# RuyiLian/CheckerPose

Measured on AMD Instinct MI355X. Metric: crops/sec forward (256x256, npt=512), higher is better.
Workload: dtype bf16; 1 GPU; LMO 'ape' hr18GNN2_res6_gnn3Skip_mlpQuery npt=512, PoseNet_GNNskip forward, deterministic random-init weights; global_batch=256, parallelism=dp1 (no forward collective), launch=hipGraph replay of 104 kernel launches

## Files before the change

### __graft_entry__.py

```python
import os
import subprocess
import sys

ROOT = os.path.dirname(os.path.abspath(__file__))
if ROOT not in sys.path:
    sys.path.insert(0, ROOT)


def build():
    csrc = os.path.join(ROOT, "checkerpose_amd", "csrc")
    subprocess.check_call(["make", "-C", csrc, "-j4", "ARCH=gfx950"])
    import checkerpose_amd
    from checkerpose_amd import _abi
    lib = _abi.load()
    assert lib.cp_version() >= 233


def smoke():
    import torch
    from oracle import checkerpose_oracle as O
    from checkerpose_amd.synthetic import build_net, det_image
    oracle_kwargs = lambda: dict(backbone="hrnet_w18", res_log2=6, init_n_graph=2, n_graph=3, local_k=2, slope=0.01,
                                 graph_slope=0.2, init_graph_slope=0.2)
    assert torch.cuda.is_available(), "smoke() needs an MI355X"
    torch.set_grad_enabled(False)
    net = build_net(seed=1)
    img = det_image(1, seed=0)
    ref, _ = O.posenet_forward(net.state_dict(), img, net.init_net.knn_idx, 512, **oracle_kwargs())
    net = net.cuda()
    out = net(img.cuda(), None)
    torch.cuda.synchronize()
    worst = 0.0
    for a, b in zip(out[:4], ref[:4]):
        worst = max(worst, float((a.cpu() - b).abs().max()))
    ids_ok = bool((out[4].cpu() == ref[4]).all() and (out[5].cpu() == ref[5]).all())
    print("smoke: max |logit - oracle| = %.3e, ids equal = %s" % (worst, ids_ok))
    assert worst <= 1e-4, worst
    assert ids_ok


if __name__ == "__main__":
    build()
    if len(sys.argv) > 1 and sys.argv[1] == "smoke":
        smoke()
```

### checkerpose_amd/_abi.py

```python
import ctypes as C
import os

_HERE = os.path.dirname(os.path.abspath(__file__))
LIB_PATH = os.environ.get("CHECKERPOSE_AMD_LIB") or os.path.join(_HERE, "libcheckerpose_hip.so")

CP_F32, CP_BF16, CP_F16 = 0, 1, 2
ACT_NONE, ACT_RELU, ACT_LEAKY = 0, 1, 2
LOSS_BCE, LOSS_L1 = 0, 1
POSE_ERR_ADD, POSE_ERR_ADI = 1, 2
BOP_ERR_MSSD, BOP_ERR_MSPD, BOP_ERR_PROJ, BOP_MAP_SMALL, BOP_MAP_LARGE = 1, 2, 4, 16, 32
BOP_MATCH_NO_LDS, BOP_MATCH_SCRATCH_MASK, BOP_SCORES_NO_LDS = 1, 2, 1


class CpConvDesc(C.Structure):
    _fields_ = [("dtype", C.c_int32), ("out_f32", C.c_int32), ("B", C.c_int32), ("H", C.c_int32), ("W", C.c_int32),
                ("Cin", C.c_int32), ("in_cstride", C.c_int32), ("in_coff", C.c_int32),
                ("R", C.c_int32), ("S", C.c_int32), ("stride", C.c_int32), ("pad", C.c_int32),
                ("Ho", C.c_int32), ("Wo", C.c_int32), ("Cout", C.c_int32), ("act", C.c_int32), ("slope", C.c_float), ("ksplit", C.c_int32),
                ("o_base", C.c_int64), ("o_sb", C.c_int64), ("o_sy", C.c_int64), ("o_sx", C.c_int64),
                ("o_sc", C.c_int64)]


_P, _I, _F, _L = C.c_void_p, C.c_int, C.c_float, C.c_longlong

# ... 30 lines not shown
                ("dw_sr", C.c_int64), ("dw_ss", C.c_int64)]


CP_BN_ITEM_STATS, CP_BN_ITEM_APPLY, CP_BN_ITEM_BWD_SUMS, CP_BN_ITEM_BWD_APPLY = 0, 1, 2, 3
BN_GROUP_MAX = 16


class CpBnItem(C.Structure):
    _fields_ = [("kind", C.c_int32), ("dtype", C.c_int32), ("blocks", C.c_uint32), ("lds_bytes", C.c_uint32),
                ("params", C.c_uint64 * 24)]


CP_WGRAD_ITEM_3X3, CP_WGRAD_ITEM_3X3_SMALL, CP_WGRAD_ITEM_GENERIC_BF16, CP_WGRAD_ITEM_GENERIC_F32 = 0, 1, 2, 3
CP_WGRAD_ITEM_3X3_S2_SMALL = 4


class CpWgradItem(C.Structure):
    _fields_ = [("kind", C.c_int32), ("blocks", C.c_uint32), ("gx", C.c_uint32), ("gy", C.c_uint32), ("params", C.c_uint64 * 20)]


class CpOptItem(C.Structure):
    _fields_ = [("p", C.c_void_p), ("g", C.c_void_p), ("m", C.c_void_p), ("v", C.c_void_p), ("n", C.c_uint64), ("step0", C.c_uint32),
                ("pad", C.c_uint32)]


class CpFuseBwdItem(C.Structure):
    _fields_ = [("dout", C.c_void_p), ("out", C.c_void_p), ("dsrc", C.c_void_p), ("Hs", C.c_int32), ("Ws", C.c_int32), ("CG", C.c_int32),
                ("shift", C.c_int32), ("relu", C.c_int32), ("accumulate", C.c_int32), ("total", C.c_uint64)]


class CpWgradDesc(C.Structure):
    _fields_ = [("dtype", C.c_int32), ("B", C.c_int32), ("H", C.c_int32), ("W", C.c_int32), ("Ho", C.c_int32),
                ("Wo", C.c_int32), ("Cout", C.c_int32), ("dy_cstride", C.c_int32), ("dy_coff", C.c_int32),
                ("Cin", C.c_int32), ("x_cstride", C.c_int32), ("x_coff", C.c_int32),
                ("R", C.c_int32), ("S", C.c_int32), ("stride", C.c_int32), ("pad", C.c_int32),
                ("dw_base", C.c_int64), ("dw_sco", C.c_int64), ("dw_sci", C.c_int64), ("dw_sr", C.c_int64),
                ("dw_ss", C.c_int64)]


SIGNATURES = {
    "cp_version": (_I, []),
    "cp_device_status": (_I, [_P, _I]),
    "cp_set_deterministic": (None, [_I]),
    "cp_get_deterministic": (_I, []),
    "cp_strerror": (C.c_char_p, [_I]),
    "cp_last_kernel": (C.c_char_p, []),
    "cp_kernel_log_begin": (None, []),
    "cp_kernel_log": (C.c_char_p, []),
    "cp_chan_align": (_I, [_I]),
    "cp_packed_weight_bytes": (C.c_size_t, [_I, _I, _I, _I, _I]),
    "cp_pack_conv_weight": (_I, [_P, _I, _P, _I, _I, _I, _I, _I, _I, _I, _P, _I, _P]),
    "cp_conv2d_igemm": (_I, [_P, C.POINTER(CpConvDesc), _P, _P, _P, _P, _P, _P]),
    "cp_conv2d_igemm_splitk": (_I, [_I, C.c_longlong, _I, _I]),
    "cp_packed_halo_weight_bytes": (C.c_size_t, [_I, _I, _I]),
    "cp_pack_conv3x3_halo_weight": (_I, [_P, _I, _P, _I, _I, _I, _P]),
    "cp_conv3x3_halo": (_I, [_P, C.POINTER(CpConvDesc), _P, _P, _P, _P, _P, _P]),
    "cp_conv2x2_halo_supported": (_I, [_I, _I, _I, _I]),
    "cp_packed_conv2x2_halo_weight_bytes": (C.c_size_t, [_I, _I, _I]),
    "cp_pack_conv2x2_halo_weight": (_I, [_P, _I, _P, _I, _I, _I, _P]),
    "cp_conv2x2_halo": (_I, [_P, C.POINTER(CpConvDesc), _P, _P, _P, _P, _P, _P]),
    "cp_conv3x3_s2_small_supported": (_I, [_I, _I, _I, _I]),
    "cp_conv3x3_s2_small_weight_bytes": (C.c_size_t, [_I, _I]),
    "cp_pack_conv3x3_s2_small_weight": (_I, [_P, _P, _I, _I, _I, _I, _P]),
    "cp_conv3x3_s2_small": (_I, [_P, C.POINTER(CpConvDesc), _P, _P, _P, _P, _P]),
    "cp_conv3x3_halo_up2x_supported": (_I, [_I, _I]),
    "cp_conv3x3_halo_up2x": (_I, [_P, C.POINTER(CpConvDesc), _P, _P, _P, _P, _P]),
    "cp_conv3x3_halo_seg_supported": (_I, [_I, _I, _I]),
    "cp_conv3x3_halo_seg": (_I, [_P, C.POINTER(CpConvDesc), _P, _P, _P, _P, _P, _P, _P, _I, _P]),
    "cp_pack_conv3x3_rows_weight": (_I, [_P, _I, _P, _I, _I, _I, _P]),
    "cp_basicblock_fused": (_I, [_P, C.POINTER(CpConvDesc), _P, _P, _P, _P, _P, _P, _P, _P]),
    "cp_bottleneck_fused": (_I, [_P, C.POINTER(CpConvDesc)] + [_P] * 14),
    "cp_packed_gemm_weight_bytes": (C.c_size_t, [_I, _I, _I]),
    "cp_pack_gemm_weight": (_I, [_P, _I, _P, _I, _I, _I, _P]),
    "cp_gemm_rows": (_I, [_P, C.POINTER(CpConvDesc), _P, _P, _P, _P, _P, _P]),
    "cp_mlp_query_fused_supported": (_I, [_I, _I, _I, _I]),
    "cp_mlp_query_fused": (_I, [_P, _P, _I, _I, _I, _I, _P, _P, _P, _F, _P, _P, _P, _F, _P, _P, _P, _L, _L, _L, _L]),
    "cp_mlp_query_fused_t": (_I, [_P, _I, _P, _I, _I, _I, _I, _P, _P, _P, _F, _P, _P, _P, _F, _P, _P, _P, _L, _L, _L, _L]),
    "cp_mlp_query_fused_n": (_I, [_P, _I, _P, _I, _I, _I, _I, _P, _P, _P, _F, _P, _P, _P, _F, _P, _P, _I, _P, _L, _L, _L, _L,
                                  _P, _P, _P, _P]),
    "cp_mlp_pair_fused_supported": (_I, [_I, _I, _I]),
    "cp_mlp_pair_fused": (_I, [_P, _P, _I, _I, _I, _I, _I, _P, _P, _F, _P, _P, _F, _P, _I, _I]),
    "cp_mlp_pair_fused_t": (_I, [_P, _I, _P, _I, _I, _I, _I, _I, _P, _P, _F, _P, _P, _F, _P, _I, _I]),
    "cp_mlp_pair_fused_gather_supported": (_I, [_I, _I, _I]),
    "cp_mlp_pair_fused_gather": (_I, [_P, C.POINTER(CpI2fGather), _P, _I, _I, _I, _I, _I, _P, _P, _F, _P, _P, _F, _P, _I, _I]),
    "cp_mlp_pair_fused_gather_t": (_I, [_P, _I, C.POINTER(CpI2fGather), _P, _I, _I, _I, _I, _I, _P, _P, _F, _P, _P, _F, _P, _I, _I]),
    "cp_hr_stem_weight_bytes": (C.c_size_t, [_I]),
    "cp_pack_hr_stem_weights": (_I, [_P, _P, _P, _P, _P]),
    "cp_hr_stem": (_I, [_P, _P, _I, _I, _I, _P, _P, _P, _P, _P, _P, _P]),
    "cp_hr_chain_supported": (_I, [_I, _I, _I]),
    "cp_hr_chain_weight_bytes": (C.c_size_t, [_I, _I, _I]),
    "cp_hr_chain_affine_floats": (_I, [_I, _I, _I]),
    "cp_pack_hr_chain_weight": (_I, [_P, _P, _P, _I, _I, _I, _I, _P]),
    "cp_hr_branch_chain": (_I, [_P, _I, _I, _I, _I, _I, C.POINTER(_P), C.POINTER(C.c_int32), _I, _P, _P, _P]),
    "cp_hr_chain_tail_supported": (_I, [_I, _I, _I]),
    "cp_hr_chain_tail_weight_bytes": (C.c_size_t, []),
    "cp_hr_chain_tail_channels": (_I, []),
    "cp_pack_hr_chain_tail_weight": (_I, [_P, _P, _P, _I, _I, _I, _P]),
    "cp_hr_branch_chain_tail": (_I, [_P, _I, _I, _I, _I, _I, C.POINTER(_P), C.POINTER(C.c_int32), _I, _P, _P, _P, C.POINTER(CpChainTail)]),
    "cp_hr_chain_tailconv_supported": (_I, [_I, _I, _I, _I, _I]),
    "cp_hr_chain_tailconv_weight_bytes": (C.c_size_t, [_I, _I, _I, _I, _I]),
    "cp_pack_hr_chain_tailconv_weight": (_I, [_P, _P, _P, _I, _I, _I, _I, _I, _P]),
    "cp_hr_branch_chain_tails": (_I, [_P, _I, _I, _I, _I, _I, C.POINTER(_P), C.POINTER(C.c_int32), _I, _P, _P, _P, _I, C.POINTER(CpChainTailConv)]),
    "cp_upsample2x_bilinear_ac": (_I, [_P, _I, _P, _P, _I, _I, _I, _I, _I, _I, _I, _I]),
    "cp_fuse_sum_act": (_I, [_P, _I, _I, C.POINTER(_P), C.POINTER(C.c_int32), _P, _I, _I, _I, _I, _I, _I, _I]),
    "cp_maxpool3x3s2": (_I, [_P, _I, _P, _P, _I, _I, _I, _I]),
    "cp_edgeconv_gather_max": (_I, [_P, _I, _P, _P, _P, _P, _I, _I, _I, _I, _I, _I, _I, _F]),
# ... 235 lines not shown
```

### checkerpose_amd/csrc/api.hip

```cpp
#include <stdarg.h>
#include <stdio.h>
#include <string.h>

#include "common.h"

extern "C" int cp_version(void) { return 233; }

std::atomic<int> g_cp_deterministic{0};
extern "C" void cp_set_deterministic(int on) { g_cp_deterministic.store(on ? 1 : 0, std::memory_order_relaxed); }
extern "C" int cp_get_deterministic(void) { return g_cp_deterministic.load(std::memory_order_relaxed); }

static std::atomic<uint32_t*> g_status_word[256];
uint32_t* cp_status_word(bool create) {
  const int dev = cp_current_device();
  if (dev < 0 || dev > 255) return nullptr;
  uint32_t* p = g_status_word[dev].load(std::memory_order_acquire);
  if (p || !create) return p;
  hipStreamCaptureStatus cs = hipStreamCaptureStatusNone;
  if (hipStreamIsCapturing(nullptr, &cs) == hipSuccess && cs != hipStreamCaptureStatusNone) return nullptr;
  uint32_t* q = nullptr;
  if (hipMalloc((void**)&q, 256) != hipSuccess) return nullptr;
  if (hipMemset(q, 0, 256) != hipSuccess) { (void)hipFree(q); return nullptr; }
  uint32_t* expect = nullptr;
  if (!g_status_word[dev].compare_exchange_strong(expect, q, std::memory_order_acq_rel)) { (void)hipFree(q); return expect; }
  return q;
}
extern "C" int cp_device_status(uint32_t* status_out, int clear) {
  if (!status_out) return CP_ERR_INVALID;
  uint32_t* p = cp_status_word(true);
  if (!p) return CP_ERR_HIP;
  if (hipMemcpy(status_out, p, sizeof(uint32_t), hipMemcpyDeviceToHost) != hipSuccess) return CP_ERR_HIP;
  if (clear && *status_out && hipMemset(p, 0, sizeof(uint32_t)) != hipSuccess) return CP_ERR_HIP;
  return CP_OK;
}

static thread_local char g_last_kernel[128] = "";
static thread_local char g_kernel_log[1024] = "";
void cp_mark_kernel(const char* fmt, ...) {
  char tmp[128];
  va_list ap;
  va_start(ap, fmt);
  vsnprintf(tmp, sizeof(tmp), fmt, ap);
  va_end(ap);
  const char* b = tmp;
  size_t n = strlen(tmp);
  if (n >= 2 && tmp[0] == '(' && tmp[n - 1] == ')') { b = tmp + 1; n -= 2; }
  memcpy(g_last_kernel, b, n);
  g_last_kernel[n] = 0;
  const size_t have = strlen(g_kernel_log);
  if (have + n + 4 < sizeof(g_kernel_log))
    snprintf(g_kernel_log + have, sizeof(g_kernel_log) - have, "%s%s", have ? " + " : "", g_last_kernel);
}
extern "C" const char* cp_last_kernel(void) { return g_last_kernel; }
extern "C" void cp_kernel_log_begin(void) { g_kernel_log[0] = 0; }
extern "C" const char* cp_kernel_log(void) { return g_kernel_log; }

extern "C" const char* cp_strerror(int code) {
  switch (code) {
    case CP_OK: return "ok";
// ... 34 lines not shown
```

### checkerpose_amd/csrc/conv_igemm.hip

```cpp
#include <stdlib.h>

#include "common.h"

struct ConvParams {
  const void* in; const void* w; const float* scale; const float* shift; const void* res; void* out;
  int M, H, W, HoWo, Wo;
  int Cin, in_cs, in_coff;
  int R, S, stride, pad;
  int KC, Cout, n_tiles, m_blocks, n_blocks, old_map;
  int act; float slope; int out_f32; int epi_lds;
  uint32_t in_bytes, w_bytes;
  long long o_base, o_sb, o_sy, o_sx, o_sc;
};

template <typename Tag> struct Mma;
template <> struct Mma<F32Tag> {
  static __device__ __forceinline__ void run(const u32x4& w, const u32x4& a, f32x4& acc) {
    acc = __builtin_amdgcn_mfma_f32_16x16x4f32(__uint_as_float(w.x), __uint_as_float(a.x), acc, 0, 0, 0);
    acc = __builtin_amdgcn_mfma_f32_16x16x4f32(__uint_as_float(w.y), __uint_as_float(a.y), acc, 0, 0, 0);
    acc = __builtin_amdgcn_mfma_f32_16x16x4f32(__uint_as_float(w.z), __uint_as_float(a.z), acc, 0, 0, 0);
    acc = __builtin_amdgcn_mfma_f32_16x16x4f32(__uint_as_float(w.w), __uint_as_float(a.w), acc, 0, 0, 0);
  }
};
template <> struct Mma<BF16Tag> {
  static __device__ __forceinline__ void run(const u32x4& w, const u32x4& a, f32x4& acc) {
    acc = __builtin_amdgcn_mfma_f32_16x16x32_bf16(__builtin_bit_cast(bf16x8, w), __builtin_bit_cast(bf16x8, a), acc, 0, 0, 0);
  }
};

template <> struct Mma<F16Tag> {
  static __device__ __forceinline__ void run(const u32x4& w, const u32x4& a, f32x4& acc) { acc = cp_mma16<true>(w, a, acc); }
};

template <typename Tag, int MT, int NT>
__global__ __launch_bounds__(256) void conv_igemm_kernel(const ConvParams p) {
  if (p.out_f32 == 2 || Tag::dtype == CP_F16) cp_f16_saturate_on();
  constexpr int E = Tag::E;
  constexpr int KCH = 4 * E;
  constexpr int ES = 16 / E;
  const int lane = threadIdx.x & 63;
  const int wave = __builtin_amdgcn_readfirstlane(threadIdx.x >> 6);
  const int x = lane & 15, q = lane >> 4;
  const int label = blockIdx.x & 7, slot = blockIdx.x >> 3;
  int nblk = slot % p.n_blocks;
  int mblk = (slot / p.n_blocks) * 8 + label;
  if (p.old_map) { const int m8 = (p.m_blocks + 7) / 8 * 8; mblk = blockIdx.x % m8; nblk = blockIdx.x / m8; }
  if (mblk >= p.m_blocks) return;
  const int m_wave = mblk * (4 * MT * 16) + wave * (MT * 16);
  const int nt0 = nblk * NT;

  int iy0[MT], ix0[MT], rowbase[MT];
#pragma unroll
  for (int mt = 0; mt < MT; ++mt) {
    const int m = m_wave + mt * 16 + x;
    const bool ok = m < p.M;
    const int mm = ok ? m : 0;
    const int b = mm / p.HoWo;
    const int rem = mm - b * p.HoWo;
    const int oy = rem / p.Wo;
    const int ox = rem - oy * p.Wo;
    iy0[mt] = ok ? oy * p.stride - p.pad : -(1 << 28);
    ix0[mt] = ox * p.stride - p.pad;
    rowbase[mt] = ((b * p.H + (ok ? iy0[mt] : 0)) * p.W + ix0[mt]) * p.in_cs + p.in_coff;
  }
  int kk = q * E;
  int tap = kk / p.Cin;
  int c = kk - tap * p.Cin;
  int r = tap / p.S;
  int s = tap - r * p.S;

  const __amdgpu_buffer_rsrc_t rsrc =
      __builtin_amdgcn_make_buffer_rsrc(const_cast<void*>(p.in), 0, p.in_bytes, 0x00020000);
  const __amdgpu_buffer_rsrc_t wrsrc =
      __builtin_amdgcn_make_buffer_rsrc(const_cast<void*>(p.w), 0, p.w_bytes, 0x00020000);
  uint32_t woff[NT];
#pragma unroll
  for (int nt = 0; nt < NT; ++nt) {
    int t = nt0 + nt;
    t = t < p.n_tiles ? t : p.n_tiles - 1;
    woff[nt] = ((uint32_t)t * p.KC * 64 + lane) * 16u;
  }

  constexpr bool EPI = (MT == 2 && (NT == 1 || NT == 2 || NT == 4));
  constexpr bool f32o = (E == 4);
  constexpr int CPL = f32o ? 4 : 8;
  constexpr int LPP = EPI ? NT * 16 / CPL : 1;
  constexpr int PPP = 64 / LPP;
  constexpr int NPASS = EPI ? MT * 16 / PPP : 1;
  const int pl0 = lane / LPP, cg = lane - pl0 * LPP;
  const int cch = nt0 * 16 + cg * CPL;
  u32x4 rres[NPASS];
  long long ofs[NPASS];
  bool okp[NPASS];
  if constexpr (EPI) if (p.epi_lds) {
    const bool cok = cch < p.Cout;
#pragma unroll
    for (int ps = 0; ps < NPASS; ++ps) {
      const int m = m_wave + ps * PPP + pl0;
      okp[ps] = (m < p.M) & cok;
      const int mm = m < p.M ? m : 0;
      const int b = mm / p.HoWo;
      const int rem = mm - b * p.HoWo;
      const int oy = rem / p.Wo;
      const int ox = rem - oy * p.Wo;
      ofs[ps] = p.o_base + (long long)b * p.o_sb + (long long)oy * p.o_sy + (long long)ox * p.o_sx + cch;
      rres[ps] = u32x4{0u, 0u, 0u, 0u};
      if (p.res && okp[ps])
        rres[ps] = f32o ? *(const u32x4*)((const float*)p.res + ofs[ps]) : *(const u32x4*)((const uint16_t*)p.res + ofs[ps]);
    }
  }

  f32x4 acc[MT][NT];
#pragma unroll
  for (int mt = 0; mt < MT; ++mt)
#pragma unroll
    for (int nt = 0; nt < NT; ++nt) acc[mt][nt] = f32x4{0.f, 0.f, 0.f, 0.f};

  const bool wide_c = p.Cin >= KCH;
  auto load_chunk = [&](u32x4* a, u32x4* w, int kc) {
    const int tapoff = (r * p.W + s) * p.in_cs + c;
    const bool tap_ok = r < p.R;
#pragma unroll
    for (int mt = 0; mt < MT; ++mt) {
      const bool ok = tap_ok & ((unsigned)(iy0[mt] + r) < (unsigned)p.H) & ((unsigned)(ix0[mt] + s) < (unsigned)p.W);
      const uint32_t off = ok ? (uint32_t)(rowbase[mt] + tapoff) * ES : 0x80000000u;
      a[mt] = __builtin_bit_cast(u32x4, __builtin_amdgcn_raw_buffer_load_b128(rsrc, off, 0, 0));
    }
#pragma unroll
    for (int nt = 0; nt < NT; ++nt)
      w[nt] = __builtin_bit_cast(u32x4, __builtin_amdgcn_raw_buffer_load_b128(wrsrc, woff[nt] + (uint32_t)kc * 1024u, 0, 0));
    c += KCH;
    if (wide_c) {
      const bool wrap = c >= p.Cin;
      c = wrap ? c - p.Cin : c;
      s += wrap ? 1 : 0;
      const bool swrap = s == p.S;
      s = swrap ? 0 : s;
      r += swrap ? 1 : 0;
    } else {
      while (c >= p.Cin) {
        c -= p.Cin;
        if (++s == p.S) { s = 0; ++r; }
      }
    }
  };
  auto compute = [&](const u32x4* a, const u32x4* w) {
#pragma unroll
    for (int mt = 0; mt < MT; ++mt)
#pragma unroll
      for (int nt = 0; nt < NT; ++nt) Mma<Tag>::run(w[nt], a[mt], acc[mt][nt]);
  };

  u32x4 a0[MT], w0[NT], a1[MT], w1[NT];
  load_chunk(a0, w0, 0);
  load_chunk(a1, w1, 1);
  for (int kc = 0; kc < p.KC; kc += 2) {
    compute(a0, w0);
    load_chunk(a0, w0, kc + 2);
    if (kc + 1 < p.KC) compute(a1, w1);
    load_chunk(a1, w1, kc + 3);
  }

  if constexpr (EPI) if (p.epi_lds) {
    extern __shared__ __attribute__((aligned(16))) float epi_smem[];
    constexpr int ROWF = NT * 16 + 4;
    float* my = epi_smem + wave * (MT * 16 * ROWF);
#pragma unroll
    for (int mt = 0; mt < MT; ++mt)
#pragma unroll
      for (int nt = 0; nt < NT; ++nt) {
        const int n = (nt0 + nt) * 16 + q * 4;
        f32x4 v = f32x4{0.f, 0.f, 0.f, 0.f};
        if (nt0 + nt < p.n_tiles && n < p.Cout) {
          const f32x4 sc = *(const f32x4*)(p.scale + n);
          const f32x4 sh = *(const f32x4*)(p.shift + n);
#pragma unroll
          for (int j = 0; j < 4; ++j) v[j] = acc[mt][nt][j] * sc[j] + sh[j];
        }
        *(f32x4*)(my + (mt * 16 + x) * ROWF + nt * 16 + q * 4) = v;
      }
    __builtin_amdgcn_s_waitcnt(0xc07f);
    __builtin_amdgcn_wave_barrier();
#pragma unroll
    for (int ps = 0; ps < NPASS; ++ps) {
      const float* src = my + (ps * PPP + pl0) * ROWF + cg * CPL;
      float v[8];
      const f32x4 v0 = *(const f32x4*)src;
      v[0] = v0[0]; v[1] = v0[1]; v[2] = v0[2]; v[3] = v0[3];
      if (!f32o) { const f32x4 v1 = *(const f32x4*)(src + 4); v[4] = v1[0]; v[5] = v1[1]; v[6] = v1[2]; v[7] = v1[3]; }
      if (!okp[ps]) continue;
      if (p.res) {
        if (f32o) {
          v[0] += __uint_as_float(rres[ps].x); v[1] += __uint_as_float(rres[ps].y);
          v[2] += __uint_as_float(rres[ps].z); v[3] += __uint_as_float(rres[ps].w);
        } else {
          float r8[8];
          Vec16<BF16Tag>::unpack(rres[ps], r8);
#pragma unroll
          for (int j = 0; j < 8; ++j) v[j] += r8[j];
        }
      }
#pragma unroll
      for (int j = 0; j < 8; ++j) {
        v[j] = cp_act_apply(v[j], cp_act_slope(p.act, p.slope));
      }
      if (f32o) *(f32x4*)((float*)p.out + ofs[ps]) = f32x4{v[0], v[1], v[2], v[3]};
      else *(u32x4*)((uint16_t*)p.out + ofs[ps]) = Vec16<BF16Tag>::pack(v);
    }
    return;
  }

  const bool vec = (p.o_sc == 1);
  const bool f32io = p.out_f32 == 1 || E == 4;
  const bool h16out = p.out_f32 == 2 || (Tag::dtype == CP_F16 && p.out_f32 == 0);
  long long pix[MT];
  bool pok[MT];
#pragma unroll
  for (int mt = 0; mt < MT; ++mt) {
    const int m = m_wave + mt * 16 + x;
// ... 22 lines not shown
                               __uint_as_float(r2.y << 16), __uint_as_float(r2.y & 0xffff0000u)};
          }
        }
      }
  }
#pragma unroll
  for (int mt = 0; mt < MT; ++mt) {
    if (!pok[mt]) continue;
#pragma unroll
    for (int nt = 0; nt < NT; ++nt) {
      const int n = (nt0 + nt) * 16 + q * 4;
      if (nt0 + nt >= p.n_tiles || n >= p.Cout) continue;
      const f32x4 sc = *(const f32x4*)(p.scale + n);
      const f32x4 sh = *(const f32x4*)(p.shift + n);
      float v[4];
#pragma unroll
      for (int j = 0; j < 4; ++j) v[j] = acc[mt][nt][j] * sc[j] + sh[j];
      if (vec) {
        const long long o = pix[mt] + n;
        if (p.res) {
#pragma unroll
          for (int j = 0; j < 4; ++j) v[j] += rv[mt][nt][j];
        }
#pragma unroll
        for (int j = 0; j < 4; ++j) {
          v[j] = cp_act_apply(v[j], cp_act_slope(p.act, p.slope));
        }
        if (f32io) {
          *(f32x4*)((float*)p.out + o) = f32x4{v[0], v[1], v[2], v[3]};
        } else if (h16out) {
          u32x2 pk; pk.x = cp_pack2<true>(v[0], v[1]); pk.y = cp_pack2<true>(v[2], v[3]);
          *(u32x2*)((uint16_t*)p.out + o) = pk;
        } else {
          u32x2 pk; pk.x = pack_bf16x2(v[0], v[1]); pk.y = pack_bf16x2(v[2], v[3]);
          *(u32x2*)((uint16_t*)p.out + o) = pk;
        }
      } else {
#pragma unroll
        for (int j = 0; j < 4; ++j) {
          if (n + j >= p.Cout) continue;
          const long long o = pix[mt] + (long long)(n + j) * p.o_sc;
          float y = v[j];
          if (p.res) y += f32io ? ((const float*)p.res)[o] : bf16_bits_to_f32(((const uint16_t*)p.res)[o]);
          y = cp_act_apply(y, cp_act_slope(p.act, p.slope));
          if (f32io) ((float*)p.out)[o] = y;
          else if (h16out) ((uint16_t*)p.out)[o] = (uint16_t)f32_to_f16_bits_sat(y);
          else ((uint16_t*)p.out)[o] = (uint16_t)f32_to_bf16_bits(y);
        }
      }
    }
  }
}

template <typename Tag, int NT, int KS>
__global__ __launch_bounds__(KS * 64) void conv_igemm_splitk_kernel(const ConvParams p) {
  if (p.out_f32 == 2 || Tag::dtype == CP_F16) cp_f16_saturate_on();
  constexpr int E = Tag::E, KCH = 4 * E, ES = 16 / E, MT = 2, T = MT * NT;
  constexpr int U = NT == 1 ? 8 : (NT == 2 ? 6 : 4);
  __shared__ __attribute__((aligned(16))) float red[KS * T * 64 * 4];
  const int lane = threadIdx.x & 63;
  const int wave = __builtin_amdgcn_readfirstlane(threadIdx.x >> 6);
  const int x = lane & 15, q = lane >> 4;
  const int nblk = blockIdx.x % p.n_blocks, mblk = blockIdx.x / p.n_blocks;
  const int m0 = mblk * (MT * 16), nt0 = nblk * NT;

  int iy0[MT], ix0[MT], rowbase[MT];
#pragma unroll
  for (int mt = 0; mt < MT; ++mt) {
    const int m = m0 + mt * 16 + x;
    const bool ok = m < p.M;
    const int mm = ok ? m : 0;
    const int b = mm / p.HoWo;
    const int rem = mm - b * p.HoWo;
    const int oy = rem / p.Wo;
    const int ox = rem - oy * p.Wo;
    iy0[mt] = ok ? oy * p.stride - p.pad : -(1 << 28);
    ix0[mt] = ox * p.stride - p.pad;
    rowbase[mt] = ((b * p.H + (ok ? iy0[mt] : 0)) * p.W + ix0[mt]) * p.in_cs + p.in_coff;
  }
  const __amdgpu_buffer_rsrc_t rsrc = __builtin_amdgcn_make_buffer_rsrc(const_cast<void*>(p.in), 0, p.in_bytes, 0x00020000);
  const __amdgpu_buffer_rsrc_t wrsrc = __builtin_amdgcn_make_buffer_rsrc(const_cast<void*>(p.w), 0, p.w_bytes, 0x00020000);
  uint32_t woff[NT];
#pragma unroll
  for (int nt = 0; nt < NT; ++nt) {
    int t = nt0 + nt;
    t = t < p.n_tiles ? t : p.n_tiles - 1;
    woff[nt] = ((uint32_t)t * p.KC * 64 + lane) * 16u;
  }
  f32x4 acc[MT][NT];
#pragma unroll
  for (int mt = 0; mt < MT; ++mt)
#pragma unroll
    for (int nt = 0; nt < NT; ++nt) acc[mt][nt] = f32x4{0.f, 0.f, 0.f, 0.f};

  for (int kc0 = wave; kc0 < p.KC; kc0 += KS * U) {
    u32x4 a[U][MT], w[U][NT];
#pragma unroll
    for (int u = 0; u < U; ++u) {
      const int kc = kc0 + u * KS;
      const int kk = kc * KCH + q * E;
      const int tap = kk / p.Cin, c = kk - tap * p.Cin;
      const int r = tap / p.S, s_ = tap - r * p.S;
      const int tapoff = (r * p.W + s_) * p.in_cs + c;
#pragma unroll
      for (int mt = 0; mt < MT; ++mt) {
        const bool ok = (r < p.R) & ((unsigned)(iy0[mt] + r) < (unsigned)p.H) & ((unsigned)(ix0[mt] + s_) < (unsigned)p.W);
// ... 67 lines not shown
      } else if (h16out) {
        u32x2 pk; pk.x = cp_pack2<true>(v[0], v[1]); pk.y = cp_pack2<true>(v[2], v[3]);
        *(u32x2*)((uint16_t*)p.out + o) = pk;
      } else {
        u32x2 pk; pk.x = pack_bf16x2(v[0], v[1]); pk.y = pack_bf16x2(v[2], v[3]);
        *(u32x2*)((uint16_t*)p.out + o) = pk;
      }
    } else {
#pragma unroll
      for (int j = 0; j < 4; ++j) {
        if (n + j >= p.Cout) continue;
        const long long o = pix + (long long)(n + j) * p.o_sc;
        float y = v[j];
        if (p.res) y += f32io ? ((const float*)p.res)[o] : bf16_bits_to_f32(((const uint16_t*)p.res)[o]);
        y = cp_act_apply(y, cp_act_slope(p.act, p.slope));
        if (f32io) ((float*)p.out)[o] = y;
        else if (h16out) ((uint16_t*)p.out)[o] = (uint16_t)f32_to_f16_bits_sat(y);
        else ((uint16_t*)p.out)[o] = (uint16_t)f32_to_bf16_bits(y);
      }
    }
  }
}

static int splitk_plan(int dtype, long long M, int KC, int n_tiles, int* NTs) {
  if ((dtype != CP_BF16 && dtype != CP_F16) || KC < 6 || cp_knob("CP_NO_SPLITK")) return 0;
  int NT = 1, best = 1 << 30;
  for (int nt = 5; nt >= 1; --nt) {
    const int padded = (n_tiles + nt - 1) / nt * nt;
    if (padded < best) { best = padded; NT = nt; }
  }
  const long long blocks2 = ((M + 127) / 128) * ((n_tiles + NT - 1) / NT);
  if (blocks2 > (KC >= 64 ? 192 : 96)) return 0;
  const long long m32 = (M + 31) / 32;
  *NTs = 1;
  for (int nt = 3; nt >= 2; --nt)
    if (m32 * ((n_tiles + nt - 1) / nt) >= 256) { *NTs = nt; break; }
  return KC >= 24 ? 8 : 4;
}

template <int NT, int KS>
static void launch_splitk(ConvParams p, hipStream_t st, bool half_in) {
  p.m_blocks = (p.M + 31) / 32;
  p.n_blocks = (p.n_tiles + NT - 1) / NT;
  cp_mark_kernel("conv_igemm_splitk_kernel<%s, %d, %d>", half_in ? "F16Tag" : "BF16Tag", NT, KS);
  if (half_in) hipLaunchKernelGGL((conv_igemm_splitk_kernel<F16Tag, NT, KS>), dim3((unsigned)(p.m_blocks * p.n_blocks)), dim3(KS * 64), 0, st, p);
  else hipLaunchKernelGGL((conv_igemm_splitk_kernel<BF16Tag, NT, KS>), dim3((unsigned)(p.m_blocks * p.n_blocks)), dim3(KS * 64), 0, st, p);
}

extern "C" int cp_conv2d_igemm_splitk(int dtype, long long M, int K, int Cout) {
  if (M <= 0 || K <= 0 || Cout <= 0 || (dtype != CP_F32 && dtype != CP_BF16 && dtype != CP_F16)) return 0;
  const int KCH = 4 * cp_chan_align(dtype);
  int nts = 1;
  return splitk_plan(dtype, M, (K + KCH - 1) / KCH, (Cout + 15) / 16, &nts);
}

template <typename Tag, int MT, int NT>
static void launch(ConvParams p, hipStream_t st) {
  p.m_blocks = (p.M + 4 * MT * 16 - 1) / (4 * MT * 16);
  p.n_blocks = (p.n_tiles + NT - 1) / NT;
  p.old_map = cp_knob("CP_OLD_MAP") ? 1 : 0;
  dim3 grid((unsigned)((p.m_blocks + 7) / 8 * 8) * p.n_blocks);
  const size_t lds = p.epi_lds ? (size_t)4 * MT * 16 * (NT * 16 + 4) * sizeof(float) : 0;
  cp_mark_kernel("conv_igemm_kernel<%s, %d, %d>", Tag::dtype == CP_BF16 ? "BF16Tag" : (Tag::dtype == CP_F16 ? "F16Tag" : "F32Tag"), MT, NT);
  hipLaunchKernelGGL((conv_igemm_kernel<Tag, MT, NT>), grid, dim3(256), lds, st, p);
}

template <typename Tag, int MT>
static void dispatch_nt(const ConvParams& p, int NT, hipStream_t st) {
  switch (NT) {
    case 1: launch<Tag, MT, 1>(p, st); break;
    case 2: launch<Tag, MT, 2>(p, st); break;
    case 3: launch<Tag, MT, 3>(p, st); break;
    case 4: launch<Tag, MT, 4>(p, st); break;
    default: launch<Tag, MT, 5>(p, st); break;
  }
}

extern "C" int cp_conv2d_igemm(cp_stream_t stream, const CpConvDesc* d, const void* in, const void* packed_w,
                               const float* scale, const float* shift, const void* residual, void* out) {
  if (!d || !in || !packed_w || !scale || !shift || !out) return CP_ERR_INVALID;
  if ((d->dtype != CP_F32 && d->dtype != CP_BF16 && d->dtype != CP_F16) || !cp_act_ok(d->act, d->slope)) return CP_ERR_INVALID;
  const bool halfish = d->dtype == CP_F16 || d->out_f32 == 2;
  if (d->out_f32 < 0 || d->out_f32 > 2 || (d->out_f32 == 2 && d->dtype != CP_BF16) || (halfish && residual)) return CP_ERR_INVALID;
  const int E = cp_chan_align(d->dtype), es = cp_elem_size(d->dtype);
  if (d->B <= 0 || d->H <= 0 || d->W <= 0 || d->Ho <= 0 || d->Wo <= 0 || d->R <= 0 || d->S <= 0 || d->stride <= 0)
    return CP_ERR_INVALID;
  if (d->Cin <= 0 || d->Cin % E || d->in_coff % E || d->in_cstride % E || d->in_coff + d->Cin > d->in_cstride)
    return CP_ERR_ALIGN;
  if (d->Cout <= 0 || (d->o_sc == 1 && d->Cout % 4)) return CP_ERR_ALIGN;
  if (!cp_aligned16(in) || !cp_aligned16(packed_w) || !cp_aligned16(scale) || !cp_aligned16(shift))
    return CP_ERR_ALIGN;
  const long long in_bytes = (long long)d->B * d->H * d->W * d->in_cstride * es;
  if (in_bytes >= (1LL << 31)) return CP_ERR_RANGE;
  const long long M = (long long)d->B * d->Ho * d->Wo;
  if (M >= (1LL << 31)) return CP_ERR_RANGE;
  if (d->o_sc == 1) {
    const int oes = d->out_f32 == 1 ? 4 : es;
    if ((d->o_base % 4) || (d->o_sb % 4) || (d->o_sy % 4) || (d->o_sx % 4)) return CP_ERR_ALIGN;
    if (((uintptr_t)out % (4 * oes)) || (residual && ((uintptr_t)residual % (4 * oes)))) return CP_ERR_ALIGN;
  }
  ConvParams p;
  p.in = in; p.w = packed_w; p.scale = scale; p.shift = shift; p.res = residual; p.out = out;
  p.M = (int)M; p.H = d->H; p.W = d->W; p.HoWo = d->Ho * d->Wo; p.Wo = d->Wo;
  p.Cin = d->Cin; p.in_cs = d->in_cstride; p.in_coff = d->in_coff;
  p.R = d->R; p.S = d->S; p.stride = d->stride; p.pad = d->pad;
  const int K = d->R * d->S * d->Cin, KCH = 4 * E;
  p.KC = (K + KCH - 1) / KCH;
  p.Cout = d->Cout; p.n_tiles = (d->Cout + 15) / 16;
  p.act = d->act; p.slope = d->slope; p.out_f32 = d->out_f32;
  p.in_bytes = (uint32_t)in_bytes;
  p.w_bytes = (uint32_t)((size_t)p.n_tiles * p.KC * 1024);
  p.o_base = d->o_base; p.o_sb = d->o_sb; p.o_sy = d->o_sy; p.o_sx = d->o_sx; p.o_sc = d->o_sc;

  int nts = 1;
  if (const int ks = d->ksplit == -1 ? 0 : splitk_plan(d->dtype, M, p.KC, p.n_tiles, &nts)) {
    hipStream_t st_ = (hipStream_t)stream;
    const bool hin = d->dtype == CP_F16;
    if (ks == 8) { if (nts == 3) launch_splitk<3, 8>(p, st_, hin); else if (nts == 2) launch_splitk<2, 8>(p, st_, hin); else launch_splitk<1, 8>(p, st_, hin); }
    else         { if (nts == 3) launch_splitk<3, 4>(p, st_, hin); else if (nts == 2) launch_splitk<2, 4>(p, st_, hin); else launch_splitk<1, 4>(p, st_, hin); }
    return cp_check_launch();
  }
  int NT = 1, best = 1 << 30;
  for (int nt = 5; nt >= 1; --nt) {
    const int padded = (p.n_tiles + nt - 1) / nt * nt;
    if (padded < best) { best = padded; NT = nt; }
  }
  const long long blocks4 = ((M + 255) / 256) * ((p.n_tiles + NT - 1) / NT);
  int MT = (blocks4 >= 512 && p.KC > 4) ? 4 : 2;
  if (const char* e = cp_knob("CP_CONV_MT")) MT = atoi(e) == 2 ? 2 : 4;
  const int oes_ = d->out_f32 == 1 ? 4 : es;
  const int cpl = 16 / oes_;
  p.epi_lds = (MT == 2 && d->o_sc == 1 && !d->out_f32 && !halfish && (NT == 1 || NT == 2 || NT == 4) && d->Cout % cpl == 0 && d->o_base % cpl == 0 &&
               d->o_sb % cpl == 0 && d->o_sy % cpl == 0 && d->o_sx % cpl == 0 && ((uintptr_t)out % 16) == 0 &&
               (!residual || ((uintptr_t)residual % 16) == 0) && !cp_knob("CP_NO_EPI_LDS")) ? 1 : 0;
  hipStream_t st = (hipStream_t)stream;
  if (d->dtype == CP_F32) { if (MT == 4) dispatch_nt<F32Tag, 4>(p, NT, st); else dispatch_nt<F32Tag, 2>(p, NT, st); }
  else if (d->dtype == CP_F16) { if (MT == 4) dispatch_nt<F16Tag, 4>(p, NT, st); else dispatch_nt<F16Tag, 2>(p, NT, st); }
  else                    { if (MT == 4) dispatch_nt<BF16Tag, 4>(p, NT, st); else dispatch_nt<BF16Tag, 2>(p, NT, st); }
  return cp_check_launch();
}
```

### include/checkerpose_hip.h

```cpp
#ifndef CHECKERPOSE_HIP_H
#define CHECKERPOSE_HIP_H

#include <stddef.h>
#include <stdint.h>

#ifdef __cplusplus
extern "C" {
#endif

typedef void* cp_stream_t;

enum { CP_F32 = 0, CP_BF16 = 1, CP_F16 = 2 };
enum { CP_ACT_NONE = 0, CP_ACT_RELU = 1, CP_ACT_LEAKY = 2 };
enum { CP_LOSS_BCE = 0, CP_LOSS_L1 = 1 };
enum {
  CP_OK = 0,
  CP_ERR_INVALID = -1,
  CP_ERR_HIP = -2,
  CP_ERR_ALIGN = -3,
  CP_ERR_RANGE = -4
};

int cp_version(void);
const char* cp_strerror(int code);
const char* cp_last_kernel(void);
void cp_kernel_log_begin(void);
const char* cp_kernel_log(void);

void cp_set_deterministic(int on);
int cp_get_deterministic(void);

enum { CP_STATUS_CHAIN0_HANDOVER = 1, CP_STATUS_CHAIN0_STAGING = 2 };
int cp_device_status(uint32_t* status_out, int clear);

int cp_chan_align(int dtype);

size_t cp_packed_weight_bytes(int dtype, int cout_rows, int cin_phys, int R, int S);
int cp_pack_conv_weight(cp_stream_t stream, int dtype, const float* w, int Cout, int Cin, int R, int S,
                        int cin_phys, int transposed, int phase, const int32_t* row_map, int cout_rows,
                        void* packed);

typedef struct CpConvDesc {
  int32_t dtype;
  int32_t out_f32;
  int32_t B, H, W;
  int32_t Cin;
  int32_t in_cstride;
  int32_t in_coff;
  int32_t R, S, stride, pad;
  int32_t Ho, Wo;
  int32_t Cout;
  int32_t act;
  float slope;
  int32_t ksplit;
  int64_t o_base, o_sb, o_sy, o_sx, o_sc;
} CpConvDesc;

int cp_conv2d_igemm(cp_stream_t stream, const CpConvDesc* d, const void* in, const void* packed_w,
                    const float* scale, const float* shift, const void* residual, void* out);
int cp_conv2d_igemm_splitk(int dtype, long long M, int K, int Cout);

size_t cp_packed_halo_weight_bytes(int dtype, int Cout, int cin_phys);
int cp_pack_conv3x3_halo_weight(cp_stream_t stream, int dtype, const float* w, int Cout, int Cin, int cin_phys,
                                void* packed);
int cp_conv3x3_halo(cp_stream_t stream, const CpConvDesc* d, const void* in, const void* packed_w,
                    const float* scale, const float* shift, const void* residual, void* out);
int cp_conv2x2_halo_supported(int dtype, int H, int W, int Cout_phys);
size_t cp_packed_conv2x2_halo_weight_bytes(int dtype, int Cout, int Cin_phys);
int cp_pack_conv2x2_halo_weight(cp_stream_t stream, int dtype, const float* w, int Cout, int Cin, int cin_phys, void* packed);
int cp_conv2x2_halo(cp_stream_t stream, const CpConvDesc* d, const void* in, const void* packed_w, const float* scale,
                    const float* shift, const void* residual, void* out);

int cp_conv3x3_halo_up2x_supported(int dtype, int Cout);
int cp_conv3x3_halo_up2x(cp_stream_t stream, const CpConvDesc* d, const void* in, const void* packed_w,
                         const float* scale, const float* shift, void* out);

int cp_conv3x3_halo_seg_supported(int dtype, int Cout, int S);
int cp_conv3x3_halo_seg(cp_stream_t stream, const CpConvDesc* d, const void* in, const void* packed_w, const float* scale,
                        const float* shift, void* out, const float* seg_w, const float* seg_b, int S, float* seg_out);

int cp_conv3x3_s2_small_supported(int H, int W, int cin_phys, int out_cphys);
size_t cp_conv3x3_s2_small_weight_bytes(int cin_phys, int out_cphys);
int cp_pack_conv3x3_s2_small_weight(cp_stream_t stream, const float* w, int Cout, int Cin, int cin_phys, int out_cphys, void* packed);
int cp_conv3x3_s2_small(cp_stream_t stream, const CpConvDesc* d, const void* in, const void* packed_w, const float* scale,
                        const float* shift, void* out);

int cp_pack_conv3x3_rows_weight(cp_stream_t stream, int dtype, const float* w, int Cout, int Cin, int cin_phys,
                                void* packed);
int cp_basicblock_fused(cp_stream_t stream, const CpConvDesc* d, const void* in, const void* packed_w1,
                        const float* scale1, const float* shift1, const void* packed_w2, const float* scale2,
                        const float* shift2, void* out);

int cp_bottleneck_fused(cp_stream_t stream, const CpConvDesc* d, const void* in, const void* packed_w1,
                        const float* scale1, const float* shift1, const void* packed_w2, const float* scale2,
                        const float* shift2, const void* packed_w3, const float* scale3, const float* shift3,
                        const void* packed_wd, const float* scaled, const float* shiftd, void* out);

size_t cp_packed_gemm_weight_bytes(int dtype, int Cout, int cin_phys);
int cp_pack_gemm_weight(cp_stream_t stream, int dtype, const float* w, int Cout, int Cin, int cin_phys, void* packed);
int cp_gemm_rows(cp_stream_t stream, const CpConvDesc* d, const void* in, const void* packed_w,
                 const float* scale, const float* shift, const void* residual, void* out);

int cp_mlp_query_fused_supported(int C0, int C1, int C2, int C3);
int cp_mlp_query_fused(cp_stream_t stream, const void* in, int in_cstride, int in_coff, int B, int N,
                       const void* packed_w1, const float* scale1, const float* shift1, float slope1,
                       const void* packed_w2, const float* scale2, const float* shift2, float slope2,
                       const float* w3, const float* b3, float* out, long long o_base, long long o_sb, long long o_sn, long long o_sc);
int cp_mlp_query_fused_t(cp_stream_t stream, int dtype, const void* in, int in_cstride, int in_coff, int B, int N,
                         const void* packed_w1, const float* scale1, const float* shift1, float slope1,
                         const void* packed_w2, const float* scale2, const float* shift2, float slope2,
                         const float* w3, const float* b3, float* out, long long o_base, long long o_sb, long long o_sn, long long o_sc);
int cp_mlp_query_fused_n(cp_stream_t stream, int dtype, const void* in, int in_cstride, int in_coff, int B, int N,
                         const void* packed_w1, const float* scale1, const float* shift1, float slope1,
// ... 548 lines not shown
```

Baseline: 24940 crops/s.

## Stage igemm conv weights through an LDS ring via DMA shared across waves

Adds a WLDS variant of the implicit-GEMM conv kernel in which each wave DMAs one weight tile into a three-slot LDS ring. After a barrier, all waves read all four weight tiles from LDS instead of each wave issuing its own global buffer loads for every tile. It is selected for deep-K convs (K ≥ 384) with NT forced to 4, aiming to cut redundant global weight traffic. In exchange it adds a __syncthreads per two-chunk stage, a larger LDS footprint, and an extra barrier before the LDS epilogue.

```diff
diff --git a/__graft_entry__.py b/__graft_entry__.py
--- a/__graft_entry__.py
+++ b/__graft_entry__.py
@@ -13,7 +13,7 @@
     import checkerpose_amd
     from checkerpose_amd import _abi
     lib = _abi.load()
-    assert lib.cp_version() >= 233
+    assert lib.cp_version() >= 234
 
 
 def smoke():
diff --git a/checkerpose_amd/_abi.py b/checkerpose_amd/_abi.py
--- a/checkerpose_amd/_abi.py
+++ b/checkerpose_amd/_abi.py
@@ -106,6 +106,7 @@
     "cp_pack_conv_weight": (_I, [_P, _I, _P, _I, _I, _I, _I, _I, _I, _I, _P, _I, _P]),
     "cp_conv2d_igemm": (_I, [_P, C.POINTER(CpConvDesc), _P, _P, _P, _P, _P, _P]),
     "cp_conv2d_igemm_splitk": (_I, [_I, C.c_longlong, _I, _I]),
+    "cp_conv2d_igemm_wlds": (_I, [_I, C.c_longlong, _I, _I]),
     "cp_packed_halo_weight_bytes": (C.c_size_t, [_I, _I, _I]),
     "cp_pack_conv3x3_halo_weight": (_I, [_P, _I, _P, _I, _I, _I, _P]),
     "cp_conv3x3_halo": (_I, [_P, C.POINTER(CpConvDesc), _P, _P, _P, _P, _P, _P]),
diff --git a/checkerpose_amd/csrc/api.hip b/checkerpose_amd/csrc/api.hip
--- a/checkerpose_amd/csrc/api.hip
+++ b/checkerpose_amd/csrc/api.hip
@@ -4,7 +4,7 @@
 
 #include "common.h"
 
-extern "C" int cp_version(void) { return 233; }
+extern "C" int cp_version(void) { return 234; }
 
 std::atomic<int> g_cp_deterministic{0};
 extern "C" void cp_set_deterministic(int on) { g_cp_deterministic.store(on ? 1 : 0, std::memory_order_relaxed); }
diff --git a/checkerpose_amd/csrc/conv_igemm.hip b/checkerpose_amd/csrc/conv_igemm.hip
--- a/checkerpose_amd/csrc/conv_igemm.hip
+++ b/checkerpose_amd/csrc/conv_igemm.hip
@@ -32,8 +32,11 @@
   static __device__ __forceinline__ void run(const u32x4& w, const u32x4& a, f32x4& acc) { acc = cp_mma16<true>(w, a, acc); }
 };
 
-template <typename Tag, int MT, int NT>
-__global__ __launch_bounds__(256) void conv_igemm_kernel(const ConvParams p) {
+constexpr int WL_D = 3, WL_G = 2;
+template <int NT> constexpr int wl_ring_bytes() { return WL_D * WL_G * NT * 1024; }
+
+template <typename Tag, int MT, int NT, bool WLDS>
+__device__ __forceinline__ void conv_igemm_tile(const ConvParams& p) {
   if (p.out_f32 == 2 || Tag::dtype == CP_F16) cp_f16_saturate_on();
   constexpr int E = Tag::E;
   constexpr int KCH = 4 * E;
@@ -126,9 +129,11 @@
       const uint32_t off = ok ? (uint32_t)(rowbase[mt] + tapoff) * ES : 0x80000000u;
       a[mt] = __builtin_bit_cast(u32x4, __builtin_amdgcn_raw_buffer_load_b128(rsrc, off, 0, 0));
     }
-#pragma unroll
-    for (int nt = 0; nt < NT; ++nt)
-      w[nt] = __builtin_bit_cast(u32x4, __builtin_amdgcn_raw_buffer_load_b128(wrsrc, woff[nt] + (uint32_t)kc * 1024u, 0, 0));
+    if constexpr (!WLDS) {
+#pragma unroll
+      for (int nt = 0; nt < NT; ++nt)
+        w[nt] = __builtin_bit_cast(u32x4, __builtin_amdgcn_raw_buffer_load_b128(wrsrc, woff[nt] + (uint32_t)kc * 1024u, 0, 0));
+    }
     c += KCH;
     if (wide_c) {
       const bool wrap = c >= p.Cin;
@@ -152,19 +157,61 @@
   };
 
   u32x4 a0[MT], w0[NT], a1[MT], w1[NT];
-  load_chunk(a0, w0, 0);
-  load_chunk(a1, w1, 1);
-  for (int kc = 0; kc < p.KC; kc += 2) {
-    compute(a0, w0);
-    load_chunk(a0, w0, kc + 2);
-    if (kc + 1 < p.KC) compute(a1, w1);
-    load_chunk(a1, w1, kc + 3);
+  if constexpr (!WLDS) {
+    load_chunk(a0, w0, 0);
+    load_chunk(a1, w1, 1);
+    for (int kc = 0; kc < p.KC; kc += 2) {
+      compute(a0, w0);
+      load_chunk(a0, w0, kc + 2);
+      if (kc + 1 < p.KC) compute(a1, w1);
+      load_chunk(a1, w1, kc + 3);
+    }
+  } else {
+    static_assert(NT == 4 && WL_G == 2, "wave w stages tile w; a stage is one trip of the two-chunk loop");
+    extern __shared__ __attribute__((aligned(16))) float epi_smem[];
+    unsigned char* const ring = (unsigned char*)epi_smem;
+    int wt = nt0 + wave;
+    wt = wt < p.n_tiles ? wt : p.n_tiles - 1;
+    const uint32_t wbase = (uint32_t)wt * p.KC * 1024u;
+    const int NS = (p.KC + 1) >> 1;
+    auto dma_stage = [&](int st, int slot) {
+      int ln = lane;
+      asm volatile("" : "+v"(ln));
+#pragma unroll
+      for (int g = 0; g < WL_G; ++g) {
+        const int kc = st * WL_G + g;
+        const uint32_t off = kc < p.KC ? wbase + (uint32_t)kc * 1024u + (uint32_t)ln * 16u : 0x80000000u;
+        cp_lds_dma16(wrsrc, off, ring + ((slot * WL_G + g) * NT + wave) * 1024);
+      }
+    };
+    int slot = 0;
+    dma_stage(0, 0);
+    load_chunk(a0, w0, 0);
+    load_chunk(a1, w1, 1);
+    for (int st = 0; st < NS; ++st) {
+      __builtin_amdgcn_s_waitcnt(0x0f70 | (2 * MT));
+      __syncthreads();
+      const unsigned char* const wb = ring + slot * (WL_G * NT * 1024) + lane * 16;
+#pragma unroll
+      for (int nt = 0; nt < NT; ++nt) {
+        w0[nt] = *(const u32x4*)(wb + nt * 1024);
+        w1[nt] = *(const u32x4*)(wb + (NT + nt) * 1024);
+      }
+      slot = slot == WL_D - 1 ? 0 : slot + 1;
+      dma_stage(st + 1, slot);
+      compute(a0, w0);
+      load_chunk(a0, w0, 2 * st + 2);
+      if (2 * st + 1 < p.KC) compute(a1, w1);
+      load_chunk(a1, w1, 2 * st + 3);
+    }
+    __builtin_amdgcn_s_waitcnt(0x0f70);
   }
 
   if constexpr (EPI) if (p.epi_lds) {
     extern __shared__ __attribute__((aligned(16))) float epi_smem[];
     constexpr int ROWF = NT * 16 + 4;
     float* my = epi_smem + wave * (MT * 16 * ROWF);
+    if constexpr (WLDS) __syncthreads();
 #pragma unroll
     for (int mt = 0; mt < MT; ++mt)
 #pragma unroll
@@ -293,6 +340,12 @@
   }
 }
 
+template <typename Tag, int MT, int NT>
+__global__ __launch_bounds__(256) void conv_igemm_kernel(const ConvParams p) { conv_igemm_tile<Tag, MT, NT, false>(p); }
+
+template <typename Tag, int MT, int NT>
+__global__ __launch_bounds__(256) void conv_igemm_wlds_kernel(const ConvParams p) { conv_igemm_tile<Tag, MT, NT, true>(p); }
+
 template <typename Tag, int NT, int KS>
 __global__ __launch_bounds__(KS * 64) void conv_igemm_splitk_kernel(const ConvParams p) {
   if (p.out_f32 == 2 || Tag::dtype == CP_F16) cp_f16_saturate_on();
@@ -466,6 +519,36 @@
   const int KCH = 4 * cp_chan_align(dtype);
   int nts = 1;
   return splitk_plan(dtype, M, (K + KCH - 1) / KCH, (Cout + 15) / 16, &nts);
+}
+
+constexpr int WLDS_MIN_K = 384;
+static int wlds_plan(int dtype, long long M, int KC, int n_tiles) {
+  const int floor_kc = WLDS_MIN_K / (4 * cp_chan_align(dtype));
+  const int min_kc = cp_knob("CP_WLDS_MIN_KC") ? atoi(cp_knob("CP_WLDS_MIN_KC")) : floor_kc;
+  if (KC < min_kc || cp_knob("CP_IGEMM_DIRECT")) return 0;
+  const int padded = (n_tiles + 3) / 4 * 4;
+  if (n_tiles < 4 || (padded - n_tiles) * 4 > n_tiles) return 0;
+  return ((M + 255) / 256) * (padded / 4) >= 512 ? 4 : 2;
+}
+
+extern "C" int cp_conv2d_igemm_wlds(int dtype, long long M, int K, int Cout) {
+  if (M <= 0 || K <= 0 || Cout <= 0 || (dtype != CP_F32 && dtype != CP_BF16 && dtype != CP_F16)) return 0;
+  if (cp_conv2d_igemm_splitk(dtype, M, K, Cout)) return 0;
+  const int KCH = 4 * cp_chan_align(dtype);
+  return wlds_plan(dtype, M, (K + KCH - 1) / KCH, (Cout + 15) / 16);
+}
+
+template <typename Tag, int MT>
+static void launch_wlds(ConvParams p, hipStream_t st) {
+  constexpr int NT = 4;
+  p.m_blocks = (p.M + 4 * MT * 16 - 1) / (4 * MT * 16);
+  p.n_blocks = (p.n_tiles + NT - 1) / NT;
+  p.old_map = 0;
+  dim3 grid((unsigned)((p.m_blocks + 7) / 8 * 8) * p.n_blocks);
+  const size_t epi = p.epi_lds ? (size_t)4 * MT * 16 * (NT * 16 + 4) * sizeof(float) : 0;
+  const size_t lds = epi > (size_t)wl_ring_bytes<NT>() ? epi : (size_t)wl_ring_bytes<NT>();
+  cp_mark_kernel("conv_igemm_wlds_kernel<%s, %d, %d>", Tag::dtype == CP_BF16 ? "BF16Tag" : (Tag::dtype == CP_F16 ? "F16Tag" : "F32Tag"), MT, NT);
+  hipLaunchKernelGGL((conv_igemm_wlds_kernel<Tag, MT, NT>), grid, dim3(256), lds, st, p);
 }
 
 template <typename Tag, int MT, int NT>
@@ -541,6 +624,8 @@
   }
   const long long blocks4 = ((M + 255) / 256) * ((p.n_tiles + NT - 1) / NT);
   int MT = (blocks4 >= 512 && p.KC > 4) ? 4 : 2;
+  const int wl = wlds_plan(d->dtype, M, p.KC, p.n_tiles);
+  if (wl) { MT = wl; NT = 4; }
   if (const char* e = cp_knob("CP_CONV_MT")) MT = atoi(e) == 2 ? 2 : 4;
   const int oes_ = d->out_f32 == 1 ? 4 : es;
   const int cpl = 16 / oes_;
@@ -548,6 +633,12 @@
                d->o_sb % cpl == 0 && d->o_sy % cpl == 0 && d->o_sx % cpl == 0 && ((uintptr_t)out % 16) == 0 &&
                (!residual || ((uintptr_t)residual % 16) == 0) && !cp_knob("CP_NO_EPI_LDS")) ? 1 : 0;
   hipStream_t st = (hipStream_t)stream;
+  if (wl) {
+    if (d->dtype == CP_F32) { if (MT == 4) launch_wlds<F32Tag, 4>(p, st); else launch_wlds<F32Tag, 2>(p, st); }
+    else if (d->dtype == CP_F16) { if (MT == 4) launch_wlds<F16Tag, 4>(p, st); else launch_wlds<F16Tag, 2>(p, st); }
+    else                    { if (MT == 4) launch_wlds<BF16Tag, 4>(p, st); else launch_wlds<BF16Tag, 2>(p, st); }
+    return cp_check_launch();
+  }
   if (d->dtype == CP_F32) { if (MT == 4) dispatch_nt<F32Tag, 4>(p, NT, st); else dispatch_nt<F32Tag, 2>(p, NT, st); }
   else if (d->dtype == CP_F16) { if (MT == 4) dispatch_nt<F16Tag, 4>(p, NT, st); else dispatch_nt<F16Tag, 2>(p, NT, st); }
   else                    { if (MT == 4) dispatch_nt<BF16Tag, 4>(p, NT, st); else dispatch_nt<BF16Tag, 2>(p, NT, st); }
diff --git a/include/checkerpose_hip.h b/include/checkerpose_hip.h
--- a/include/checkerpose_hip.h
+++ b/include/checkerpose_hip.h
@@ -59,6 +59,8 @@
 int cp_conv2d_igemm(cp_stream_t stream, const CpConvDesc* d, const void* in, const void* packed_w,
                     const float* scale, const float* shift, const void* residual, void* out);
 int cp_conv2d_igemm_splitk(int dtype, long long M, int K, int Cout);
+
+int cp_conv2d_igemm_wlds(int dtype, long long M, int K, int Cout);
 
 size_t cp_packed_halo_weight_bytes(int dtype, int Cout, int cin_phys);
 int cp_pack_conv3x3_halo_weight(cp_stream_t stream, int dtype, const float* w, int Cout, int Cin, int cin_phys,
```

After: 24770 crops/s (median of 3 runs). No clear change (-0.7%).
